# earthspecies/avex

Measured on AMD Instinct MI355X. Metric: clips/s (10 s @ 16 kHz) embedding extraction, BEATs-base, higher is better.
Workload: dtype f16; 1 GPU; BEATs-base (12L/768/3072/12H, 90.7 M params, synthetic weights), batch 256 x 10 s @ 16 kHz per GPU, wav resident in HBM -> mean-pooled 768-d embedding; global_batch=256, samples_per_clip=160000, parallelism=dp1, world_size=1, inputs=avex_amd.synth.noise_clips(seed=0), keyed by global clip index, chunk_clips=256, streams=1, residual_stream=half, layernorm_fold=True

## Files before the change

avex_amd/csrc/posconv.hip:

```cpp
#include "common.h"

namespace {

constexpr int CG = 48;
constexpr int KT = 128;
constexpr int PAD = KT / 2;
constexpr int TMAX = 512;
constexpr int SLAB_ROWS = TMAX + KT;
constexpr int SLAB_BYTES = SLAB_ROWS * CG * 2;
constexpr int KTOT = KT * CG;
constexpr int NU = KT / 2;
constexpr int WST = CG * 96 * 2;
constexpr int PC_LDS = SLAB_BYTES + 2 * WST;

static __device__ __forceinline__ void pc_dma16(const void* src, const char* lds_dst) {
    const unsigned lds = (unsigned)(__UINTPTR_TYPE__)(__attribute__((address_space(3))) const char*)lds_dst;
    asm volatile("s_mov_b32 m0, %1\n\tglobal_load_lds_dwordx4 %0, off" ::"v"(src), "s"(lds) : "memory");
}

template <typename T>
__global__ __launch_bounds__(512) __attribute__((amdgpu_waves_per_eu(4, 4)))
void posconv_kernel(const T* __restrict__ xh, const float* __restrict__ xf, const T* __restrict__ wp,
                    const float* __restrict__ bias, int Tn, int E, int G, int nseg, float* __restrict__ out, T* __restrict__ out_h) {
    extern __shared__ __attribute__((aligned(16))) char slab[];
    typedef typename Half<T>::v8 v8;
    char* wring = slab + SLAB_BYTES;
    const int tid = threadIdx.x, lane = tid & 63;
    const int wave = __builtin_amdgcn_readfirstlane(tid >> 6);
    const int g = blockIdx.x % G, bs = blockIdx.x / G;
    const int b = bs / nseg, t0 = (bs - b * nseg) * TMAX;
    const T* xg = xh + (int64_t)b * Tn * E + g * CG;
    const char* wg = (const char*)(wp + (int64_t)g * CG * KTOT);

    auto issue_w = [&](int u) __attribute__((always_inline)) {
        const char* src = wg + (int64_t)u * WST;
        char* dst = wring + (u & 1) * WST;
        pc_dma16(src + wave * 1024 + lane * 16, dst + wave * 1024);
        if (wave == (u & 7)) pc_dma16(src + 8 * 1024 + lane * 16, dst + 8 * 1024);
    };
    issue_w(0);

    for (int idx = tid; idx < SLAB_ROWS * 6; idx += 512) {
        const int r = idx / 6, c = idx - r * 6;
        const int t = t0 + r - PAD;
        uint4 v = make_uint4(0, 0, 0, 0);
        if (t >= 0 && t < Tn) v = *(const uint4*)(xg + (int64_t)t * E + c * 8);
        *(uint4*)(slab + r * (CG * 2) + c * 16) = v;
    }
    asm volatile("s_waitcnt vmcnt(0)" ::: "memory");
    __syncthreads();

    const int t16 = lane & 15, g4 = lane >> 4;
    const int tw0 = wave * 64;
    const bool has_work = t0 + tw0 < Tn;

    int xoff[3];
#pragma unroll
    for (int v = 0; v < 3; ++v) {
        const int off = 32 * v + 8 * g4;
        xoff[v] = (off / CG) * (CG * 2) + (off % CG) * 2;
    }
    const char* xbase = slab + (tw0 + t16) * (CG * 2);
    const int woff = (g4 * CG + t16) * 16;

    f32x4 acc[3][4];
#pragma unroll
    for (int ot = 0; ot < 3; ++ot)
#pragma unroll
        for (int tt = 0; tt < 4; ++tt) acc[ot][tt] = (f32x4){0.f, 0.f, 0.f, 0.f};

    for (int u = 0; u < NU; ++u) {
        if (u + 1 < NU) issue_w(u + 1);
        if (has_work) {
            const char* xu = xbase + u * (2 * CG * 2);
            const char* ws = wring + (u & 1) * WST + woff;
#pragma unroll
            for (int v = 0; v < 3; ++v) {
                v8 xfr[4], wf[3];
#pragma unroll
                for (int ot = 0; ot < 3; ++ot) wf[ot] = *(const v8*)(ws + (v * 4 * CG + ot * 16) * 16);
#pragma unroll
                for (int tt = 0; tt < 4; ++tt) xfr[tt] = *(const v8*)(xu + tt * 16 * (CG * 2) + xoff[v]);
#pragma unroll
                for (int ot = 0; ot < 3; ++ot)
#pragma unroll
                    for (int tt = 0; tt < 4; ++tt) acc[ot][tt] = mfma16(wf[ot], xfr[tt], acc[ot][tt]);
            }
        }
        asm volatile("s_waitcnt vmcnt(0) lgkmcnt(0)" ::: "memory");
        __builtin_amdgcn_s_barrier();
    }
    if (!has_work) return;

    AVX_F16_SAT_BEGIN();
#pragma unroll
    for (int tt = 0; tt < 4; ++tt) {
        const int tl = tw0 + tt * 16 + t16, t = t0 + tl;
        if (t >= Tn) continue;
        const int64_t rowoff = ((int64_t)b * Tn + t) * E + g * CG;
#pragma unroll
        for (int ot = 0; ot < 3; ++ot) {
            const int n = ot * 16 + 4 * g4;
            f32x4 v = acc[ot][tt] + *(const f32x4*)(bias + g * CG + n);
            v = gelu_erf4(v);
            f32x4 r;
            if (xf) {
                r = *(const f32x4*)(xf + rowoff + n);
            } else {
                const typename Half<T>::v4 rh = *(const typename Half<T>::v4*)(slab + (tl + PAD) * (CG * 2) + n * 2);
                r = (f32x4){(float)rh[0], (float)rh[1], (float)rh[2], (float)rh[3]};
            }
            r += v;
            if (out) *(f32x4*)(out + rowoff + n) = r;
            if (out_h) {
                typename Half<T>::v4 h;
                h[0] = Half<T>::from_hw(r[0]); h[1] = Half<T>::from_hw(r[1]);
                h[2] = Half<T>::from_hw(r[2]); h[3] = Half<T>::from_hw(r[3]);
                *(typename Half<T>::v4*)(out_h + rowoff + n) = h;
            }
        }
    }
}

__global__ __launch_bounds__(256) void posconv_norm_kernel(const float* __restrict__ v, int n_rows, int K,
                                                           float* __restrict__ norm) {
    __shared__ float red[4];
    const int k = blockIdx.x;
    float s = 0.f;
    for (int r = threadIdx.x; r < n_rows; r += 256) {
        const float x = v[(int64_t)r * K + k];
        s += x * x;
    }
    s = wave_sum(s);
    if ((threadIdx.x & 63) == 0) red[threadIdx.x >> 6] = s;
    __syncthreads();
    if (threadIdx.x == 0) norm[k] = sqrtf((red[0] + red[1]) + (red[2] + red[3]));
}

template <typename T>
__global__ void posconv_pack_kernel(const float* __restrict__ v, const float* __restrict__ gk,
                                    const float* __restrict__ norm, int E, int cg, int K, T* __restrict__ out) {
    const int64_t total = (int64_t)E * cg * K;
    const int64_t i = (int64_t)blockIdx.x * blockDim.x + threadIdx.x;
    if (i >= total) return;
    const int c = (int)(i % cg);
    const int tap = (int)((i / cg) % K);
    const int64_t o = i / ((int64_t)cg * K);
    const float w = v[(o * cg + c) * K + tap] * (gk[tap] / norm[tap]);
    const int k = tap * cg + c, u = k / 96, rem = k - 96 * u, cv = rem >> 5, g4 = (rem >> 3) & 3, e = rem & 7;
    const int64_t grp = o / cg, ol = o - grp * cg;
    const int nu = cg * K / 96;
    out[(((((grp * nu + u) * 3 + cv) * 4 + g4) * cg + ol) << 3) + e] = Half<T>::from(w);
}

}

namespace avx {

int posconv_pack(const float* g, const float* v, int E, int groups, int K, void* w_packed, int dtype,
                 hipStream_t s) {
    AVX_REQUIRE(g && v && w_packed, "posconv_pack: null argument");
    AVX_REQUIRE(groups > 0 && E % groups == 0 && K > 0, "posconv_pack: bad shape E=%d groups=%d K=%d", E, groups, K);
    const int cg = E / groups;
    float* norm = nullptr;
    AVX_HIP_CHECK(hipMalloc((void**)&norm, sizeof(float) * K));
    hipLaunchKernelGGL(posconv_norm_kernel, dim3(K), dim3(256), 0, s, v, E * cg, K, norm);
    const int64_t total = (int64_t)E * cg * K;
    const dim3 grid((unsigned)((total + 255) / 256));
    if (dtype == AVEXHIP_BF16)
        hipLaunchKernelGGL(posconv_pack_kernel<__bf16>, grid, dim3(256), 0, s, v, g, norm, E, cg, K, (__bf16*)w_packed);
    else
        hipLaunchKernelGGL(posconv_pack_kernel<_Float16>, grid, dim3(256), 0, s, v, g, norm, E, cg, K, (_Float16*)w_packed);
    hipError_t e = hipGetLastError();
    hipError_t e2 = hipStreamSynchronize(s);
    (void)hipFree(norm);
    if (e != hipSuccess || e2 != hipSuccess) {
        avexhip_set_error("posconv_pack: %s", hipGetErrorString(e != hipSuccess ? e : e2));
        return AVEXHIP_ERR_HIP;
    }
    return AVEXHIP_OK;
}

int posconv(const void* x_half, const float* x_f32, const void* w_packed, const float* bias, int B, int T,
            int E, int groups, int K, float* out, void* out_half, int dtype, hipStream_t s) {
    AVX_REQUIRE(x_half && w_packed && bias && (out || out_half), "posconv: null argument");
    AVX_REQUIRE(groups > 0 && E % groups == 0 && E / groups == CG && K == KT,
                "posconv: only %d channels/group and %d taps are built (got E=%d groups=%d K=%d)", CG, KT, E, groups, K);
    AVX_REQUIRE(B > 0 && T > 0, "posconv: empty input B=%d T=%d", B, T);
    const int nseg = (T + TMAX - 1) / TMAX;
    if (dtype == AVEXHIP_BF16) {
        AVX_ENSURE_LDS(posconv_kernel<__bf16>, PC_LDS);
        hipLaunchKernelGGL(posconv_kernel<__bf16>, dim3(B * nseg * groups), dim3(512), PC_LDS, s, (const __bf16*)x_half, x_f32,
                           (const __bf16*)w_packed, bias, T, E, groups, nseg, out, (__bf16*)out_half);
    } else if (dtype == AVEXHIP_F16) {
        AVX_ENSURE_LDS(posconv_kernel<_Float16>, PC_LDS);
        hipLaunchKernelGGL(posconv_kernel<_Float16>, dim3(B * nseg * groups), dim3(512), PC_LDS, s, (const _Float16*)x_half, x_f32,
                           (const _Float16*)w_packed, bias, T, E, groups, nseg, out, (_Float16*)out_half);
    } else {
        avexhip_set_error("posconv: unknown dtype %d", dtype);
        return AVEXHIP_ERR_INVALID;
    }
    AVX_LAUNCH_CHECK();
    return AVEXHIP_OK;
}

}
```

Measured before the change: 10000 clips/s.

## Widen posconv per-wave time tile and reorder tap walk to reuse x fragments

```diff
diff --git a/avex_amd/csrc/posconv.hip b/avex_amd/csrc/posconv.hip
--- a/avex_amd/csrc/posconv.hip
+++ b/avex_amd/csrc/posconv.hip
@@ -12,19 +12,26 @@
 constexpr int NU = KT / 2;
 constexpr int WST = CG * 96 * 2;
 constexpr int PC_LDS = SLAB_BYTES + 2 * WST;
-
-static __device__ __forceinline__ void pc_dma16(const void* src, const char* lds_dst) {
-    const unsigned lds = (unsigned)(__UINTPTR_TYPE__)(__attribute__((address_space(3))) const char*)lds_dst;
-    asm volatile("s_mov_b32 m0, %1\n\tglobal_load_lds_dwordx4 %0, off" ::"v"(src), "s"(lds) : "memory");
+constexpr int NTB = 8;
+constexpr int NWAVE = TMAX / (16 * NTB);
+constexpr int NTHR = NWAVE * 64;
+constexpr int NCLS = 8;
+static __device__ __forceinline__ constexpr int cls_of(int r) { return (r + NCLS / 2) & (NCLS - 1); }
+static_assert(NCLS * NCLS == NU && NWAVE == 4, "the tap-pair walk and the weight split over the waves assume this");
+static_assert((NWAVE - 1) * 16 * NTB + 15 + 16 * (NTB - 1 + NCLS - 1) + 2 * (NCLS - 1) + 1 == SLAB_ROWS - 2, "slab read bound");
+
+static __device__ __forceinline__ void pc_dma16(const char* src_uniform, unsigned lane_off, unsigned lds_dst) {
+    asm volatile("s_mov_b32 m0, %2\n\tglobal_load_lds_dwordx4 %0, %1" ::"v"(lane_off), "s"(src_uniform), "s"(lds_dst) : "memory");
 }
 
 template <typename T>
-__global__ __launch_bounds__(512) __attribute__((amdgpu_waves_per_eu(4, 4)))
+__global__ __launch_bounds__(NTHR) __attribute__((amdgpu_waves_per_eu(NWAVE / 2, NWAVE / 2)))
 void posconv_kernel(const T* __restrict__ xh, const float* __restrict__ xf, const T* __restrict__ wp,
                     const float* __restrict__ bias, int Tn, int E, int G, int nseg, float* __restrict__ out, T* __restrict__ out_h) {
     extern __shared__ __attribute__((aligned(16))) char slab[];
     typedef typename Half<T>::v8 v8;
     char* wring = slab + SLAB_BYTES;
+    const unsigned wring_lds = (unsigned)(__UINTPTR_TYPE__)(__attribute__((address_space(3))) const char*)slab + SLAB_BYTES;
     const int tid = threadIdx.x, lane = tid & 63;
     const int wave = __builtin_amdgcn_readfirstlane(tid >> 6);
     const int g = blockIdx.x % G, bs = blockIdx.x / G;
@@ -32,15 +39,17 @@
     const T* xg = xh + (int64_t)b * Tn * E + g * CG;
     const char* wg = (const char*)(wp + (int64_t)g * CG * KTOT);
 
-    auto issue_w = [&](int u) __attribute__((always_inline)) {
-        const char* src = wg + (int64_t)u * WST;
-        char* dst = wring + (u & 1) * WST;
-        pc_dma16(src + wave * 1024 + lane * 16, dst + wave * 1024);
-        if (wave == (u & 7)) pc_dma16(src + 8 * 1024 + lane * 16, dst + 8 * 1024);
+    auto issue_w = [&](int i) __attribute__((always_inline)) {
+        const int u = cls_of(i >> 3) + NCLS * (i & (NCLS - 1));
+        const char* src = wg + u * WST;
+        const unsigned dst = wring_lds + (i & 1) * WST;
+        pc_dma16(src + wave * 1024, lane * 16, dst + wave * 1024);
+        pc_dma16(src + (NWAVE + wave) * 1024, lane * 16, dst + (NWAVE + wave) * 1024);
+        if (wave == (i & (NWAVE - 1))) pc_dma16(src + 8 * 1024, lane * 16, dst + 8 * 1024);
     };
     issue_w(0);
 
-    for (int idx = tid; idx < SLAB_ROWS * 6; idx += 512) {
+    for (int idx = tid; idx < SLAB_ROWS * 6; idx += NTHR) {
         const int r = idx / 6, c = idx - r * 6;
         const int t = t0 + r - PAD;
         uint4 v = make_uint4(0, 0, 0, 0);
@@ -51,8 +60,15 @@
     __syncthreads();
 
     const int t16 = lane & 15, g4 = lane >> 4;
-    const int tw0 = wave * 64;
-    const bool has_work = t0 + tw0 < Tn;
+    const int tw0 = wave * (16 * NTB);
+    if (t0 + tw0 >= Tn) {
+        for (int i = 0; i < NU; ++i) {
+            if (i + 1 < NU) issue_w(i + 1);
+            asm volatile("s_waitcnt vmcnt(0)" ::: "memory");
+            __builtin_amdgcn_s_barrier();
+        }
+        return;
+    }
 
     int xoff[3];
 #pragma unroll
@@ -63,38 +79,48 @@
     const char* xbase = slab + (tw0 + t16) * (CG * 2);
     const int woff = (g4 * CG + t16) * 16;
 
-    f32x4 acc[3][4];
+    f32x4 acc[3][NTB];
 #pragma unroll
     for (int ot = 0; ot < 3; ++ot)
 #pragma unroll
-        for (int tt = 0; tt < 4; ++tt) acc[ot][tt] = (f32x4){0.f, 0.f, 0.f, 0.f};
-
-    for (int u = 0; u < NU; ++u) {
-        if (u + 1 < NU) issue_w(u + 1);
-        if (has_work) {
-            const char* xu = xbase + u * (2 * CG * 2);
-            const char* ws = wring + (u & 1) * WST + woff;
+        for (int tt = 0; tt < NTB; ++tt) acc[ot][tt] = (f32x4){0.f, 0.f, 0.f, 0.f};
+
+    for (int r = 0; r < NCLS; ++r) {
+        const char* xr = xbase + cls_of(r) * (2 * CG * 2);
+        v8 xfr[3][NTB];
+#pragma unroll
+        for (int q = 0; q < NCLS; ++q) {
+            const int i = r * NCLS + q;
+            if (i + 1 < NU) issue_w(i + 1);
+            const char* ws = wring + (q & 1) * WST + woff;
+            if (q == 0) {
+#pragma unroll
+                for (int v = 0; v < 3; ++v)
+#pragma unroll
+                    for (int tt = 0; tt < NTB; ++tt) xfr[v][tt] = *(const v8*)(xr + tt * 16 * (CG * 2) + xoff[v]);
+            } else {
+#pragma unroll
+                for (int v = 0; v < 3; ++v)
+                    xfr[v][(q + NTB - 1) % NTB] = *(const v8*)(xr + (q + NTB - 1) * 16 * (CG * 2) + xoff[v]);
+            }
 #pragma unroll
             for (int v = 0; v < 3; ++v) {
-                v8 xfr[4], wf[3];
+                v8 wf[3];
 #pragma unroll
                 for (int ot = 0; ot < 3; ++ot) wf[ot] = *(const v8*)(ws + (v * 4 * CG + ot * 16) * 16);
 #pragma unroll
-                for (int tt = 0; tt < 4; ++tt) xfr[tt] = *(const v8*)(xu + tt * 16 * (CG * 2) + xoff[v]);
-#pragma unroll
-                for (int ot = 0; ot < 3; ++ot)
-#pragma unroll
-                    for (int tt = 0; tt < 4; ++tt) acc[ot][tt] = mfma16(wf[ot], xfr[tt], acc[ot][tt]);
-            }
+                for (int tt = 0; tt < NTB; ++tt)
+#pragma unroll
+                    for (int ot = 0; ot < 3; ++ot) acc[ot][tt] = mfma16(wf[ot], xfr[v][(tt + q) % NTB], acc[ot][tt]);
+            }
+            asm volatile("s_waitcnt vmcnt(0) lgkmcnt(0)" ::: "memory");
+            __builtin_amdgcn_s_barrier();
         }
-        asm volatile("s_waitcnt vmcnt(0) lgkmcnt(0)" ::: "memory");
-        __builtin_amdgcn_s_barrier();
-    }
-    if (!has_work) return;
+    }
 
     AVX_F16_SAT_BEGIN();
 #pragma unroll
-    for (int tt = 0; tt < 4; ++tt) {
+    for (int tt = 0; tt < NTB; ++tt) {
         const int tl = tw0 + tt * 16 + t16, t = t0 + tl;
         if (t >= Tn) continue;
         const int64_t rowoff = ((int64_t)b * Tn + t) * E + g * CG;
@@ -190,11 +216,11 @@
     const int nseg = (T + TMAX - 1) / TMAX;
     if (dtype == AVEXHIP_BF16) {
         AVX_ENSURE_LDS(posconv_kernel<__bf16>, PC_LDS);
-        hipLaunchKernelGGL(posconv_kernel<__bf16>, dim3(B * nseg * groups), dim3(512), PC_LDS, s, (const __bf16*)x_half, x_f32,
+        hipLaunchKernelGGL(posconv_kernel<__bf16>, dim3(B * nseg * groups), dim3(NTHR), PC_LDS, s, (const __bf16*)x_half, x_f32,
                            (const __bf16*)w_packed, bias, T, E, groups, nseg, out, (__bf16*)out_half);
     } else if (dtype == AVEXHIP_F16) {
         AVX_ENSURE_LDS(posconv_kernel<_Float16>, PC_LDS);
-        hipLaunchKernelGGL(posconv_kernel<_Float16>, dim3(B * nseg * groups), dim3(512), PC_LDS, s, (const _Float16*)x_half, x_f32,
+        hipLaunchKernelGGL(posconv_kernel<_Float16>, dim3(B * nseg * groups), dim3(NTHR), PC_LDS, s, (const _Float16*)x_half, x_f32,
                            (const _Float16*)w_packed, bias, T, E, groups, nseg, out, (_Float16*)out_half);
     } else {
         avexhip_set_error("posconv: unknown dtype %d", dtype);
```

Measured after the change: 10030 clips/s (median of 4 runs). About the same (+0.2%).
